# samyak0210/ViNet

Hardware: AMD Instinct MI355X
Metric: clips/sec training (32x224x384 bf16) (higher is better)
Workload: dtype bf16; 1 GPU; ViNet DHF1K training, 32x224x384 bf16, 192 clip(s)/GPU/step, kldiv + fused Adam, 1xMI355X; global_batch=192, local_batch=192, parallelism=dp1

## Files before the change

vinet_amd/csrc/options.h:

```cpp
#pragma once
#define VN_OPTIONS(VN_OPT) \
  VN_OPT(dma,          1, "LDS-DMA conv kernel (conv_dma) where legal; 0 = the register-staged kernel") \
  VN_OPT(dma3,         1, "LDS-DMA kernel for the split-bf16 form (conv_dma3); 0 = the register-staged kernel") \
  VN_OPT(pp,           1, "256x256x64 ping-pong conv kernel: 0 off, 1 heuristic, 2 force, 3 / 4 force the 256- / 192-wide shape") \
  VN_OPT(pp_pw_kt,     8, "ping-pong kernel on pointwise layers from this many K tiles of 64 (16 = as for every other layer)") \
  VN_OPT(pw,           1, "pointwise streaming kernel (conv_pw) for 1x1x1 convs and their data gradients: 0 off, 1 heuristic, 2 also on small grids (tests)") \
  VN_OPT(pw_maxtn,     4, "pointwise kernel: at most this many column tiles (each re-reads x)") \
  VN_OPT(ht,           1, "halo-tile conv kernels (conv_ht): 0 off, 1 heuristic, 2 every eligible conv (tests)") \
  VN_OPT(ht3,          1, "halo-tile kernels for the split-bf16 form; 0 = conv_dma3 everywhere") \
  VN_OPT(ht_minhw,     28 * 48, "halo tiles, spatial mode: smallest H x W the heuristic takes") \
  VN_OPT(ht_t,         1, "temporal mode of the halo-tile kernel for (3,1,1) / stride-1 convs; 0 off") \
  VN_OPT(ht_t_minhw,   14 * 24, "halo tiles, temporal mode: smallest H x W the heuristic takes") \
  VN_OPT(ht_pre,       0, "halo tiles, spatial mode, on inputs with a pending BatchNorm + ReLU: 1 on") \
  VN_OPT(conv_hs,      1, "strip-streaming kernel of the folded stem (conv_hs): 0 off, 1 heuristic, 2 every eligible shape (tests)") \
  VN_OPT(conv_hs_segs, 1, "conv_hs: row segments for launches on small grids; 0 = whole strips only") \
  VN_OPT(conv_ts,      1, "frame-streaming temporal 64 -> 64 kernels (conv_ts, conv_tsd): 0 off, 1 heuristic, 2 every eligible shape (tests)") \
  VN_OPT(conv_ts_segs, 1, "conv_ts: frame segments for launches on small grids; 0 = whole patches only") \
  VN_OPT(splitk,       1, "split-K on grids that cannot fill the chip: 0 off, 1 on, n >= 2 = minimum K chunks (of 32) per split") \
  VN_OPT(sk_tile,      7, "tiles of long-K small-grid convs whose caller lends split-K scratch: bit 0 128x192, bit 1 128x128, bit 2 / 3 128x64 / 256x64") \
  VN_OPT(n64_tile,     0, "tuning: 64-wide layers on 128x64 (1) or 64x64 (2) tiles instead of 256x64") \
  VN_OPT(n64_kmax,     64, "64-wide outputs: 128-row tiles up to this many K steps of 32 (0 = never)") \
  VN_OPT(n128_tile,    0, "tuning: 128-wide layers on 128x128 (1) or 64x128 (2) tiles instead of 256x128") \
  VN_OPT(n128_kmax,    64, "128-wide outputs: 128-row tiles up to this many K steps of 32 (0 = never)") \
  VN_OPT(n192_tile,    1, "128x192 tiles for N % 192 == 0 instead of 256x96: 0 off, 1 heuristic, 2 also on small grids (tests)") \
  VN_OPT(tperm,        0, "t-fastest M-tile order (L2 reuse across temporal taps): 1 on") \
  VN_OPT(epi_rows,     0, "conv epilogue stores whole rows through a wave-private LDS image: 1 on (-DVINET_EXPERIMENTS builds only)") \
  VN_OPT(bnb_epi,      1, "BatchNorm-backward partial sums out of the shared conv epilogue; 0 = only the fused temporal data gradient") \
  VN_OPT(wgrad_dma,    1, "LDS-DMA multi-tap weight-gradient kernel where legal; 0 = the register-staged kernel") \
  VN_OPT(wgrad_tg,     0, "tuning: taps per group in the LDS-DMA weight gradient (0 = heuristic)") \
  VN_OPT(wgrad_tr,     1, "hardware transpose reads in the register-staged weight gradient; 0 = scalar LDS reads") \
  VN_OPT(wgrad_pp,     1, "256x256x64 ping-pong weight gradient: 0 off, 1 heuristic, 2 force, 3 / 4 force the 256- / 192-row tile") \
  VN_OPT(wgrad_pp_cap, 1, "the ping-pong weight gradient honours VinetWgradDesc::max_cus; 0 = always the whole chip") \
  VN_OPT(wgrad_ts,     1, "frame-streaming weight gradient of temporal 64 -> 64 convs: 0 off, 1 heuristic, 2 every eligible shape (tests)") \
  VN_OPT(wgrad_ts_cap, 0, "the frame-streaming weight gradient honours VinetWgradDesc::max_cus: 1 on") \
  VN_OPT(wgrad_hs,     1, "strip-streaming weight gradient of the folded stem: 0 off, 1 heuristic, 2 every eligible shape (tests)") \
  VN_OPT(wgrad_rs,     1, "row-streaming weight gradient of 1x3x3 convs: 0 off, 1 heuristic, 2 every eligible shape (tests)") \
  VN_OPT(wgrad_rs4,    1, "row-streaming weight gradient: the four-wave form for W = 24, 48, 32, 64, 96; 0 = the eight-wave kernels") \
  VN_OPT(wgrad_tf,     1, "temporal-tap weight gradient (wgrad_tf): 0 off, 1 heuristic, 2 every eligible shape (tests)") \
  VN_OPT(wgrad_skinny, 1, "weight gradient of pointwise convs with 8 output channels: 0 off, 1 heuristic, 2 every eligible shape (tests)") \
  VN_OPT(bn_lean,      1, "register-lean bf16 BatchNorm-backward kernels: 0 = the generic 8-channel forms, 2 = a -DVINET_EXPERIMENTS variant") \
  VN_OPT(bn_rows,      1024, "cap on the workgroups (= partial rows) of a channel reduction (clamped to >= 1)") \
  VN_OPT(reduce_il,    1, "channel reductions: blocks interleave rounds over one window; 0 = one contiguous range per block") \
  VN_OPT(reduce_small, 1, "tensors of <= 64 voxels take channel_reduce_small_kernel; 0 off") \
  VN_OPT(pack_tiled,   1, "LDS-tiled multi-tensor pack / unpack; 0 = the element-wise kernels") \
  VN_OPT(pool_lds,     1, "LDS halo-tile 3x3x3/s1 max-pool forward (C % 64 == 0): 0 off, 1 large tensors, 2 always") \
  VN_OPT(pool_pk,      1, "bf16: packed 32-bit-key form of the LDS halo-tile pool; 0 = the fp32-compare kernel") \
  VN_OPT(pool_twalk,   1, "T-walking 3x3x3/s1 max-pool backward: 0 off, 1 large tensors, 2 always (any value above 3 too), 3 conditional-load form.  The forward's 8-channel T-walking kernel (kT 3, sT 1) reads it too: >= 2 forces it on small tensors, 0 does NOT switch it off") \
  VN_OPT(pool_blk,     1, "strided max-pool backward per 2x2 input block; 0 off") \
  VN_OPT(up_blk,       1, "8-channel upsample kernels (forward per 2x2 output block); 0 off") \
  VN_OPT(auc_ws,       0, "AUC-Judd sorts and counts in the caller's workspace whatever the number of fixations: 1 on (tests); 0 = in LDS up to 4096 fixations") \
  VN_OPT(sauc_ws,      0, "shuffled AUC reads the other-fixation list from the caller's workspace whatever its length: 1 on (tests); 0 = staged in LDS up to 8192 locations")

#define VN_OPT_DECLARE(name, dflt, text) extern int g_vinet_opt_##name;
VN_OPTIONS(VN_OPT_DECLARE)
```

vinet_amd/csrc/pool.hip:

```cpp
#include "elementwise.h"

struct PoolP { int kT, kH, kW, sT, sH, sW, pT, pH, pW; FastDiv dsT, dsH, dsW; };
static inline PoolP make_poolp(const VinetPoolDesc* d) {
  PoolP p = {d->kT, d->kH, d->kW, d->sT, d->sH, d->sW, d->pT, d->pH, d->pW, make_fastdiv((uint32_t)d->sT), make_fastdiv((uint32_t)d->sH), make_fastdiv((uint32_t)d->sW)};
  return p;
}

template <typename T> VN_DEV float pool_round(float v) { return v; }
template <> VN_DEV float pool_round<bf16_t>(float v) { return bf2f(f2bf(v)); }
template <typename T> VN_DEV float4 pool_pre4(float4 v, const Affine& pre, int c) {
  v = affine4(v, pre, c);
  if (pre.scale) { v.x = pool_round<T>(v.x); v.y = pool_round<T>(v.y); v.z = pool_round<T>(v.z); v.w = pool_round<T>(v.w); }
  return v;
}
template <typename T> VN_DEV float pool_pre(float f, float sc, float sh, const Affine& pre) {
  float v = fmaf(f, sc, sh);
  if (pre.relu) v = fmaxf(v, 0.f);
  if (pre.scale) v = pool_round<T>(v);
  return v;
}
VN_DEV void pool_column(const TView& v, uint32_t col, int& b, int& h, int& w) {
  const uint32_t r1 = fdiv(col, v.dW);
  w = (int)(col - r1 * (uint32_t)v.W);
  const uint32_t r2 = fdiv(r1, v.dH);
// ... 400 lines not shown
  const int h0 = th * 8, w0 = tw * 8, c0 = cg * 64 + oct * 8;
  const int ho = h0 + ph, wo = w0 + pw;
  const bool out_ok = ho < y.H && wo < y.W && c0 < x.C;
  const bool aff = pre.scale != nullptr;
  if (tid < 64) {
    const bool ok = aff && cg * 64 + tid < x.C;
    S[0][tid] = ok ? pre.scale[cg * 64 + tid] : 1.f;
    S[1][tid] = ok ? pre.shift[cg * 64 + tid] : 0.f;
  }
  __syncthreads();
  uint32_t m_a[8], m_b[8], m_c[8];
#pragma unroll
  for (int e = 0; e < 8; ++e) { m_a[e] = 0; m_b[e] = 0; m_c[e] = 0; }
  const int T_ = x.T;
  for (int tp = 0; tp <= T_; ++tp) {
    uint16_t (*buf)[64] = P[tp & 1];
    if (tp < T_) {
      for (int it = tid; it < 800; it += 512) {
        const int hp = it >> 3;
        const int hh = h0 - 1 + hp / 10, ww = w0 - 1 + hp % 10;
        if (cg * 64 + oct * 8 >= x.C) continue;
        uint4 q = make_uint4(0, 0, 0, 0);
        if ((unsigned)hh < (unsigned)x.H && (unsigned)ww < (unsigned)x.W) {
          q = *(const uint4*)((const bf16_t*)x.p + vox_off(x, b, tp, hh, ww) + cg * 64 + oct * 8);
          if (aff) {
            const float2* sp = (const float2*)&S[0][oct * 8];
            const float2* hp2 = (const float2*)&S[1][oct * 8];
            uint32_t* w4 = (uint32_t*)&q;
#pragma unroll
            for (int e = 0; e < 4; ++e) {
              const float2 s2 = sp[e], h2 = hp2[e];
              if (pre.relu) w4[e] = pre_relu_pair(w4[e], (f32x2_v){s2.x, s2.y}, (f32x2_v){h2.x, h2.y});
              else w4[e] = pack2bf(fmaf(__uint_as_float(w4[e] << 16), s2.x, h2.x), fmaf(__uint_as_float(w4[e] & 0xffff0000u), s2.y, h2.y));
            }
          } else if (pre.relu) {
            uint32_t* w4 = (uint32_t*)&q;
#pragma unroll
            for (int e = 0; e < 4; ++e) asm("v_pk_max_i16 %0, %1, 0" : "=v"(w4[e]) : "v"(w4[e]));
          }
          q.x = pool_code2(q.x); q.y = pool_code2(q.y); q.z = pool_code2(q.z); q.w = pool_code2(q.w);
        }
        *(uint4*)&buf[hp][oct * 8] = q;
      }
    }
    __syncthreads();
#pragma unroll
    for (int e = 0; e < 8; ++e) { m_a[e] = m_b[e]; m_b[e] = m_c[e]; m_c[e] = 0; }
    if (tp < T_) {
#pragma unroll
      for (int kh = 0; kh < 3; ++kh)
#pragma unroll
        for (int kw = 0; kw < 3; ++kw) {
          const uint4 q = *(const uint4*)&buf[(ph + kh) * 10 + pw + kw][oct * 8];
          const uint32_t ck = 8u - (uint32_t)(kh * 3 + kw);
          const uint32_t w4[4] = {q.x, q.y, q.z, q.w};
#pragma unroll
          for (int e = 0; e < 4; ++e) {
            const uint32_t klo = (w4[e] << 16) | ck, khi = (w4[e] & 0xffff0000u) | ck;
            m_c[2 * e] = m_c[2 * e] > klo ? m_c[2 * e] : klo;
            m_c[2 * e + 1] = m_c[2 * e + 1] > khi ? m_c[2 * e + 1] : khi;
          }
        }
    }
    const int to = tp - 1;
    if (to < 0 || !out_ok) continue;
    uint32_t ov[4];
    unsigned long long oi = 0;
    const bool va = to >= 1, vc = to + 1 < T_;
#pragma unroll
    for (int e = 0; e < 8; ++e) {
      const uint32_t ka = va ? m_a[e] + 18u : 0u, kb = m_b[e] + 9u, kc = vc ? m_c[e] : 0u;
      uint32_t k = ka > kb ? ka : kb;
      k = k > kc ? k : kc;
      if (e & 1) ov[e >> 1] |= k & 0xffff0000u; else ov[e >> 1] = k >> 16;
      oi |= (unsigned long long)(26u - (k & 0xffu)) << (8 * e);
    }
    uint4 o;
    o.x = pool_decode2(ov[0]); o.y = pool_decode2(ov[1]); o.z = pool_decode2(ov[2]); o.w = pool_decode2(ov[3]);
    *(uint4*)((bf16_t*)y.p + vox_off(y, b, to, ho, wo) + c0) = o;
    if (argmax) {
      const long ovox = (((long)b * y.T + to) * y.H + ho) * y.W + wo;
      *(unsigned long long*)(argmax + ovox * y.C + c0) = oi;
    }
  }
}

#define POOL_ADD_IF_X(g, word, BYTE, code, v, exec0)                                                                                  \
  asm volatile("v_cmpx_eq_u32_sdwa vcc, %1, %2 src0_sel:BYTE_" #BYTE " src1_sel:DWORD\n\tv_add_f32_e32 %0, %0, %3\n\ts_mov_b64 exec, %4" \
               : "+v"(g) : "v"(word), "s"(code), "v"(v), "s"(exec0) : "vcc")
#define POOL_ADD_IF(g, word, BYTE, code, v) POOL_ADD_IF_X(g, word, BYTE, code, v, exec0)
#define POOL_ADD_IF8(g, lo, hi, e, code, v, ex)                                           \
  do {                                                                                      \
    const uint32_t w_ = (e) < 4 ? (lo) : (hi);                                              \
    switch ((e) & 3) {                                                                      \
      case 0: POOL_ADD_IF_X(g, w_, 0, code, v, ex); break;                                  \
      case 1: POOL_ADD_IF_X(g, w_, 1, code, v, ex); break;                                  \
      case 2: POOL_ADD_IF_X(g, w_, 2, code, v, ex); break;                                  \
      default: POOL_ADD_IF_X(g, w_, 3, code, v, ex); break;                                 \
    }                                                                                       \
  } while (0)

template <typename T>
__global__ void maxpool_bwd_kernel(PoolP p, TView dy, const uint8_t* __restrict__ argmax, TView dx, int accumulate,
                                   long total) {
  const long i = (long)blockIdx.x * blockDim.x + threadIdx.x;
  if (i >= total) return;
  const uint32_t vox_u = fdiv((uint32_t)i, dx.dQ);
  const int q = (int)((uint32_t)i - vox_u * (uint32_t)(dx.C / 4));
  const long vox = (long)vox_u;
  int b, t, h, w;
  decode_vox(dx, vox, b, t, h, w);
  float g[4] = {0, 0, 0, 0};
  const int to1 = min((int)fdiv((uint32_t)(t + p.pT), p.dsT), dy.T - 1), ho1 = min((int)fdiv((uint32_t)(h + p.pH), p.dsH), dy.H - 1),
            wo1 = min((int)fdiv((uint32_t)(w + p.pW), p.dsW), dy.W - 1);
  const int to0 = (int)fdiv((uint32_t)max(0, t + p.pT - p.kT + p.sT), p.dsT), ho0 = (int)fdiv((uint32_t)max(0, h + p.pH - p.kH + p.sH), p.dsH),
            wo0 = (int)fdiv((uint32_t)max(0, w + p.pW - p.kW + p.sW), p.dsW);
  for (int to = to0; to <= to1; ++to) {
    const int kt = t + p.pT - to * p.sT;
    if (kt < 0 || kt >= p.kT) continue;
    for (int ho = ho0; ho <= ho1; ++ho) {
      const int kh = h + p.pH - ho * p.sH;
      if (kh < 0 || kh >= p.kH) continue;
      for (int wo = wo0; wo <= wo1; ++wo) {
        const int kw = w + p.pW - wo * p.sW;
        if (kw < 0 || kw >= p.kW) continue;
        const uint32_t tap = (uint32_t)((kt * p.kH + kh) * p.kW + kw);
        const long ovox = (((long)b * dy.T + to) * dy.H + ho) * dy.W + wo;
        const uint32_t am = *(const uint32_t*)(argmax + ovox * dy.C + q * 4);
        const uint32_t xr = am ^ (tap * 0x01010101u);
        if (!((xr - 0x01010101u) & ~xr & 0x80808080u)) continue;
        const float4 d = ldq<T>((const T*)dy.p + vox_off(dy, b, to, ho, wo) + q * 4);
        if ((xr & 0xffu) == 0) g[0] += d.x;
        if ((xr & 0xff00u) == 0) g[1] += d.y;
        if ((xr & 0xff0000u) == 0) g[2] += d.z;
        if ((xr & 0xff000000u) == 0) g[3] += d.w;
      }
    }
  }
  T* dst = (T*)dx.p + vox_off(dx, b, t, h, w) + q * 4;
  if (accumulate) { const float4 o = ldq<T>(dst); g[0] += o.x; g[1] += o.y; g[2] += o.z; g[3] += o.w; }
  stq<T>(dst, make_float4(g[0], g[1], g[2], g[3]));
}

template <typename T>
__global__ __launch_bounds__(256) void maxpool_bwd_k3s1_kernel(TView dy, const uint8_t* __restrict__ argmax, TView dx,
                                                               int accumulate, long total) {
  const long i = (long)blockIdx.x * blockDim.x + threadIdx.x;
  if (i >= total) return;
  const int G = dx.C >> 3;
  const uint32_t vox_u = (uint32_t)(i / G);
  const int g = (int)(i - (long)vox_u * G);
  int b, t, h, w;
  decode_vox(dx, (long)vox_u, b, t, h, w);
  const int T_ = dx.T, H = dx.H, W = dx.W;
  const long am_c = (long)vox_u * dx.C + g * 8;
  const long dy_c = vox_off(dy, b, t, h, w) + g * 8;
  unsigned long long am[27];
#pragma unroll
  for (int kt = 0; kt < 3; ++kt)
#pragma unroll
    for (int kh = 0; kh < 3; ++kh)
#pragma unroll
      for (int kw = 0; kw < 3; ++kw) {
        const int dt = 1 - kt, dh = 1 - kh, dw = 1 - kw;
        const bool ok = (unsigned)(t + dt) < (unsigned)T_ && (unsigned)(h + dh) < (unsigned)H && (unsigned)(w + dw) < (unsigned)W;
        const long d = ((long)(dt * H + dh) * W + dw) * (long)dx.C;
// ... 63 lines not shown
      }
    }
  }
  T* dst = (T*)dx.p + vox_off(dx, b, t, h, w) + g * 8;
  if (accumulate) {
    float o[8];
    ld8<T>(dst, o);
#pragma unroll
    for (int e = 0; e < 8; ++e) gr[e] += o[e];
  }
  st8<T>(dst, gr);
}

template <typename T>
__global__ __launch_bounds__(256) void maxpool_bwd_k133s2_kernel(TView dy, const uint8_t* __restrict__ argmax, TView dx, int accumulate,
                                                                 int HB, int WB, long total) {
  const long i = (long)blockIdx.x * blockDim.x + threadIdx.x;
  if (i >= total) return;
  const int G = dx.C >> 3;
  long r = i / G;
  const int g = (int)(i - r * G);
  const int wb = (int)(r % WB); r /= WB;
  const int hb = (int)(r % HB); r /= HB;
  const int t = (int)(r % dx.T);
  const int b = (int)(r / dx.T);
  const int h0 = 2 * hb, w0 = 2 * wb;
  unsigned long long am[4];
  bool wok[4];
#pragma unroll
  for (int q = 0; q < 4; ++q) {
    const int ho = hb + (q >> 1), wo = wb + (q & 1);
    wok[q] = ho < dy.H && wo < dy.W;
    const long ovox = (((long)b * dy.T + t) * dy.H + (wok[q] ? ho : 0)) * dy.W + (wok[q] ? wo : 0);
    am[q] = wok[q] ? *(const unsigned long long*)(argmax + ovox * dy.C + g * 8) : ~0ull;
  }
  float dv[4][8];
#pragma unroll
  for (int q = 0; q < 4; ++q) {
    bool any = false;
#pragma unroll
    for (int kh = 0; kh < 3; ++kh)
#pragma unroll
      for (int kw = 0; kw < 3; ++kw) {
        const bool in = ((q >> 1) ? kh == 0 : kh >= 1) && ((q & 1) ? kw == 0 : kw >= 1);
        if (!in) continue;
        const unsigned long long x = am[q] ^ ((unsigned long long)(kh * 3 + kw) * 0x0101010101010101ull);
        any |= ((x - 0x0101010101010101ull) & ~x & 0x8080808080808080ull) != 0;
      }
    if (any) ld8<T>((const T*)dy.p + vox_off(dy, b, t, hb + (q >> 1), wb + (q & 1)) + g * 8, dv[q]);
    else {
#pragma unroll
      for (int e = 0; e < 8; ++e) dv[q][e] = 0.f;
    }
  }
#pragma unroll
  for (int ih = 0; ih < 2; ++ih)
#pragma unroll
    for (int iw = 0; iw < 2; ++iw) {
      const int h = h0 + ih, w = w0 + iw;
      if (h >= dx.H || w >= dx.W) continue;
      float gr[8] = {0, 0, 0, 0, 0, 0, 0, 0};
      unsigned long long ex;
      asm volatile("s_mov_b64 %0, exec" : "=s"(ex));
#pragma unroll
      for (int q = 0; q < 4; ++q) {
        const int dh = q >> 1, dw = q & 1;
        const int kh = ih + 1 - 2 * dh, kw = iw + 1 - 2 * dw;
        if (kh < 0 || kw < 0) continue;
        const uint32_t alo = (uint32_t)am[q], ahi = (uint32_t)(am[q] >> 32);
#pragma unroll
        for (int e = 0; e < 8; ++e) POOL_ADD_IF8(gr[e], alo, ahi, e, (uint32_t)(kh * 3 + kw), dv[q][e], ex);
      }
      T* dst = (T*)dx.p + vox_off(dx, b, t, h, w) + g * 8;
      if (accumulate) {
        float o[8];
        ld8<T>(dst, o);
#pragma unroll
        for (int e = 0; e < 8; ++e) gr[e] += o[e];
      }
      st8<T>(dst, gr);
    }
}

template <typename T>
__global__ __launch_bounds__(256) void maxpool_bwd_k3s2_kernel(TView dy, const uint8_t* __restrict__ argmax, TView dx, int accumulate,
                                                               int TB, int HB, int WB, long total) {
  const long i = (long)blockIdx.x * blockDim.x + threadIdx.x;
  if (i >= total) return;
  const int G = dx.C >> 3;
  long r = i / G;
  const int g = (int)(i - r * G);
  const int wb = (int)(r % WB); r /= WB;
  const int hb = (int)(r % HB); r /= HB;
  const int tb = (int)(r % TB);
  const int b = (int)(r / TB);
  unsigned long long am[8];
  float dv[8][8];
#pragma unroll
  for (int w = 0; w < 8; ++w) {
    const int to = tb + (w >> 2), ho = hb + ((w >> 1) & 1), wo = wb + (w & 1);
    const bool ok = to < dy.T && ho < dy.H && wo < dy.W;
    am[w] = ~0ull;
    if (ok) {
      const long ovox = (((long)b * dy.T + to) * dy.H + ho) * dy.W + wo;
      am[w] = *(const unsigned long long*)(argmax + ovox * dy.C + g * 8);
      ld8<T>((const T*)dy.p + vox_off(dy, b, to, ho, wo) + g * 8, dv[w]);
    } else {
#pragma unroll
      for (int e = 0; e < 8; ++e) dv[w][e] = 0.f;
    }
  }
#pragma unroll
  for (int v = 0; v < 8; ++v) {
    const int it = v >> 2, ih = (v >> 1) & 1, iw = v & 1;
    const int t = 2 * tb + it, h = 2 * hb + ih, w_ = 2 * wb + iw;
    if (t >= dx.T || h >= dx.H || w_ >= dx.W) continue;
    float gr[8] = {0, 0, 0, 0, 0, 0, 0, 0};
    unsigned long long ex;
    asm volatile("s_mov_b64 %0, exec" : "=s"(ex));
#pragma unroll
    for (int w = 0; w < 8; ++w) {
      const int dt = w >> 2, dh = (w >> 1) & 1, dw = w & 1;
      if (dt > it || dh > ih || dw > iw) continue;
      const int kt = dt ? 0 : it + 1, kh = dh ? 0 : ih + 1, kw = dw ? 0 : iw + 1;
      const uint32_t alo = (uint32_t)am[w], ahi = (uint32_t)(am[w] >> 32);
#pragma unroll
      for (int e = 0; e < 8; ++e) POOL_ADD_IF8(gr[e], alo, ahi, e, (uint32_t)((kt * 3 + kh) * 3 + kw), dv[w][e], ex);
    }
    T* dst = (T*)dx.p + vox_off(dx, b, t, h, w_) + g * 8;
    if (accumulate) {
      float o[8];
      ld8<T>(dst, o);
#pragma unroll
      for (int e = 0; e < 8; ++e) gr[e] += o[e];
    }
    st8<T>(dst, gr);
  }
}

template <typename T>
__global__ __launch_bounds__(256) void maxpool_bwd_k3s1_twalk_kernel(TView dy, const uint8_t* __restrict__ argmax, TView dx,
                                                                     int accumulate, long total) {
  const long i = (long)blockIdx.x * blockDim.x + threadIdx.x;
  if (i >= total) return;
  const int G = dx.C >> 3;
  const uint32_t col = (uint32_t)(i / G);
  const int g = (int)(i - (long)col * G);
  int b, h, w;
  pool_column(dx, col, b, h, w);
  const int T_ = dx.T, H = dx.H, W = dx.W;
  float g_m[8], g_0[8], g_p[8];
#pragma unroll
  for (int e = 0; e < 8; ++e) { g_m[e] = 0.f; g_0[e] = 0.f; g_p[e] = 0.f; }
  for (int to = 0; to <= T_; ++to) {
    if (to < T_) {
      unsigned long long am[9];
#pragma unroll
      for (int kh = 0; kh < 3; ++kh)
#pragma unroll
        for (int kw = 0; kw < 3; ++kw) {
          const int ho = h + 1 - kh, wo = w + 1 - kw;
          const bool ok = (unsigned)ho < (unsigned)H && (unsigned)wo < (unsigned)W;
          const long ovox = (((long)b * T_ + to) * H + (ok ? ho : 0)) * W + (ok ? wo : 0);
          am[kh * 3 + kw] = ok ? *(const unsigned long long*)(argmax + ovox * dx.C + g * 8) : ~0ull;
        }
#pragma unroll
// ... 25 lines not shown
#pragma unroll
        for (int e = 0; e < 8; ++e) g_m[e] += o[e];
      }
      st8<T>(dst, g_m);
    }
#pragma unroll
    for (int e = 0; e < 8; ++e) { g_m[e] = g_0[e]; g_0[e] = g_p[e]; g_p[e] = 0.f; }
  }
}

__global__ __launch_bounds__(256) void maxpool_bwd_k3s1_tw3_kernel(TView dy, const uint8_t* __restrict__ argmax, TView dx,
                                                                   int accumulate, long total) {
  const long i = (long)blockIdx.x * blockDim.x + threadIdx.x;
  if (i >= total) return;
  unsigned long long exec0;
  asm volatile("s_mov_b64 %0, exec" : "=s"(exec0));
  const int G = dx.C >> 3;
  const uint32_t col = (uint32_t)(i / G);
  const int g = (int)(i - (long)col * G);
  int b, h, w;
  pool_column(dx, col, b, h, w);
  const int T_ = dx.T, H = dx.H, W = dx.W;
  const uint8_t* amp = argmax + ((((long)b * T_) * H + h) * W + w) * (long)dx.C + g * 8;
  const unsigned short* dyp = (const unsigned short*)dy.p + vox_off(dy, b, 0, h, w) + g * 8;
  const long am_plane = (long)H * W * dx.C, dy_plane = (long)H * W * dy.ld;
  uint32_t okmask = 0;
#pragma unroll
  for (int kh = 0; kh < 3; ++kh)
#pragma unroll
    for (int kw = 0; kw < 3; ++kw) {
      const int ho = h + 1 - kh, wo = w + 1 - kw;
      okmask |= (((unsigned)ho < (unsigned)H && (unsigned)wo < (unsigned)W) ? 1u : 0u) << (kh * 3 + kw);
    }
  float g_m[8], g_0[8], g_p[8];
#pragma unroll
  for (int e = 0; e < 8; ++e) { g_m[e] = 0.f; g_0[e] = 0.f; g_p[e] = 0.f; }
  for (int to = 0; to <= T_; ++to) {
    if (to < T_) {
      unsigned long long am[9];
      uint4 dv[9];
#pragma unroll
      for (int s = 0; s < 9; ++s) {
        const int dvox = (1 - s / 3) * W + (1 - s % 3);
        const bool ok = (okmask >> s) & 1u;
        am[s] = *(const unsigned long long*)(amp + (ok ? dvox * dx.C : 0));
        dv[s] = *(const uint4*)(dyp + (ok ? dvox * dy.ld : 0));
      }
#pragma unroll
      for (int s = 0; s < 9; ++s) {
        const unsigned long long a = ((okmask >> s) & 1u) ? am[s] : ~0ull;
        const uint32_t alo = (uint32_t)a, ahi = (uint32_t)(a >> 32);
        const uint32_t q[4] = {dv[s].x, dv[s].y, dv[s].z, dv[s].w};
#pragma unroll
        for (int e = 0; e < 8; ++e) {
          const uint32_t word = (e < 4) ? alo : ahi;
          const float v = (e & 1) ? __uint_as_float(q[e >> 1] & 0xffff0000u) : __uint_as_float(q[e >> 1] << 16);
          switch (e & 3) {
            case 0: POOL_ADD_IF(g_m[e], word, 0, (uint32_t)s, v); POOL_ADD_IF(g_0[e], word, 0, (uint32_t)(s + 9), v); POOL_ADD_IF(g_p[e], word, 0, (uint32_t)(s + 18), v); break;
            case 1: POOL_ADD_IF(g_m[e], word, 1, (uint32_t)s, v); POOL_ADD_IF(g_0[e], word, 1, (uint32_t)(s + 9), v); POOL_ADD_IF(g_p[e], word, 1, (uint32_t)(s + 18), v); break;
            case 2: POOL_ADD_IF(g_m[e], word, 2, (uint32_t)s, v); POOL_ADD_IF(g_0[e], word, 2, (uint32_t)(s + 9), v); POOL_ADD_IF(g_p[e], word, 2, (uint32_t)(s + 18), v); break;
            default: POOL_ADD_IF(g_m[e], word, 3, (uint32_t)s, v); POOL_ADD_IF(g_0[e], word, 3, (uint32_t)(s + 9), v); POOL_ADD_IF(g_p[e], word, 3, (uint32_t)(s + 18), v); break;
          }
        }
      }
      amp += am_plane;
      dyp += dy_plane;
    }
    const int t = to - 1;
    if (t >= 0) {
      unsigned short* dst = (unsigned short*)dx.p + vox_off(dx, b, t, h, w) + g * 8;
      if (accumulate) {
        float o[8];
        ld8<unsigned short>(dst, o);
#pragma unroll
        for (int e = 0; e < 8; ++e) g_m[e] += o[e];
      }
      st8<unsigned short>(dst, g_m);
    }
#pragma unroll
    for (int e = 0; e < 8; ++e) { g_m[e] = g_0[e]; g_0[e] = g_p[e]; g_p[e] = 0.f; }
  }
}

enum PoolKind { POOL_FWD, POOL_TSLIDE, POOL_FWD8, POOL_FWD8_PK, POOL_TSLIDE8, POOL_K3S1_LDS, POOL_K3S1_PK,
                POOL_BWD, POOL_BWD8, POOL_BWD_K133S2, POOL_BWD_K3S2, POOL_BWD_K3S1, POOL_BWD_K3S1_TWALK, POOL_BWD_K3S1_TW3 };
struct PoolRoute {
  PoolKind kind;
  const char* name;
  bool typed;
  long n;
  int tilesH, tilesW;
  int TB, HB, WB;
};

static const long POOL_FILL_COLS = 65536;

static bool pool_is_k3s1(const VinetPoolDesc* d, const VinetTensor& a, const VinetTensor& b) {
  return d->kT == 3 && d->kH == 3 && d->kW == 3 && d->sT == 1 && d->sH == 1 && d->sW == 1 && d->pT == 1 && d->pH == 1 && d->pW == 1 &&
         a.T == b.T && a.H == b.H && a.W == b.W;
}
static bool pool_oct(const VinetTensor& a, const VinetTensor& b, const uint8_t* argmax) {
  return oct_ok(a) && oct_ok(b) && ((uintptr_t)argmax % 8) == 0;
}

static PoolRoute pool_fwd_route(const VinetPoolDesc* d, const VinetTensor* x, VinetAffine pre, const VinetTensor* y, const uint8_t* argmax) {
  const bool oct = pool_oct(*x, *y, argmax);
  const bool walk_t = d->kT == 3 && d->sT == 1 && d->pT == 1 && y->T == x->T && x->T >= 2;
  const bool pk = d->dtype == VINET_BF16 && g_vinet_opt_pool_pk && (!pre.scale || pre.shift);
  const long cols8 = (long)y->B * y->H * y->W * (y->C / 8);
  if (pool_is_k3s1(d, *x, *y) && walk_t && oct && g_vinet_opt_pool_lds && (g_vinet_opt_pool_lds >= 2 || cols8 >= POOL_FILL_COLS)) {
    const int tilesH = (y->H + 7) / 8, tilesW = (y->W + 7) / 8;
    const long blocks = (long)y->B * tilesH * tilesW * ((y->C + 63) / 64);
    if (pk) return {POOL_K3S1_PK, "maxpool_k3s1_pk_kernel", false, blocks, tilesH, tilesW};
    return {POOL_K3S1_LDS, "maxpool_k3s1_lds_kernel", true, blocks, tilesH, tilesW};
  }
  if (walk_t && oct && (g_vinet_opt_pool_twalk >= 2 || cols8 >= POOL_FILL_COLS)) return {POOL_TSLIDE8, "maxpool_tslide8_kernel", true, cols8};
  if (walk_t && !(oct_ok(*x) && oct_ok(*y))) return {POOL_TSLIDE, "maxpool_tslide_kernel", true, (long)y->B * y->H * y->W * (y->C / 4)};
  if (oct) {
    const long total8 = view_voxels(*y) * (y->C / 8);
    if (pk) return {POOL_FWD8_PK, "maxpool_fwd8_pk_kernel", false, total8};
    return {POOL_FWD8, "maxpool_fwd8_kernel", true, total8};
  }
  return {POOL_FWD, "maxpool_fwd_kernel", true, view_voxels(*y) * (y->C / 4)};
}

static PoolRoute pool_bwd_route(const VinetPoolDesc* d, const VinetTensor* dy, const uint8_t* argmax, const VinetTensor* dx) {
  const bool oct = pool_oct(*dx, *dy, argmax);
  const long total8 = view_voxels(*dx) * (dx->C / 8);
  if (oct && pool_is_k3s1(d, *dx, *dy)) {
    const long cols8 = (long)dx->B * dx->H * dx->W * (dx->C / 8);
    if (g_vinet_opt_pool_twalk >= 2 || (g_vinet_opt_pool_twalk && cols8 >= POOL_FILL_COLS)) {
      if (g_vinet_opt_pool_twalk != 3 && d->dtype == VINET_BF16 && (long)dx->H * dx->W * dx->C < (1l << 30) &&
          (long)dx->H * dx->W * dy->ld < (1l << 30))
        return {POOL_BWD_K3S1_TW3, "maxpool_bwd_k3s1_tw3_kernel", false, cols8};
      return {POOL_BWD_K3S1_TWALK, "maxpool_bwd_k3s1_twalk_kernel", true, cols8};
    }
    return {POOL_BWD_K3S1, "maxpool_bwd_k3s1_kernel", true, total8};
  }
  if (oct && g_vinet_opt_pool_blk && d->kH == 3 && d->kW == 3 && d->sH == 2 && d->sW == 2 && d->pH == 1 && d->pW == 1 &&
      dy->H == (dx->H - 1) / 2 + 1 && dy->W == (dx->W - 1) / 2 + 1) {
    const int TB = (dx->T + 1) / 2, HB = (dx->H + 1) / 2, WB = (dx->W + 1) / 2;
    if (d->kT == 1 && d->sT == 1 && d->pT == 0 && dy->T == dx->T)
      return {POOL_BWD_K133S2, "maxpool_bwd_k133s2_kernel", true, (long)dx->B * dx->T * HB * WB * (dx->C / 8), 0, 0, 0, HB, WB};
    if (d->kT == 3 && d->sT == 2 && d->pT == 1 && dy->T == (dx->T - 1) / 2 + 1)
      return {POOL_BWD_K3S2, "maxpool_bwd_k3s2_kernel", true, (long)dx->B * TB * HB * WB * (dx->C / 8), 0, 0, TB, HB, WB};
  }
  if (oct) return {POOL_BWD8, "maxpool_bwd8_kernel", true, total8};
  return {POOL_BWD, "maxpool_bwd_kernel", true, view_voxels(*dx) * (dx->C / 4)};
}

static int pool_fwd_args(const VinetPoolDesc* d, const VinetTensor* x, const VinetTensor* y) {
  VN_CHECK_ARG(d && x && y && quad_ok(*x, esize(d->dtype)) && quad_ok(*y, esize(d->dtype)) && x->C == y->C && x->B == y->B,
               "maxpool3d: bad views");
  VN_CHECK_ARG(d->kT * d->kH * d->kW <= 255 && d->kT > 0 && d->kH > 0 && d->kW > 0, "maxpool3d: window too large");
  return 0;
}
static int pool_bwd_args(const VinetPoolDesc* d, const VinetTensor* dy, const uint8_t* argmax, const VinetTensor* dx) {
  VN_CHECK_ARG(d && dy && dx && argmax && quad_ok(*dy, esize(d->dtype)) && quad_ok(*dx, esize(d->dtype)) &&
                   dx->C == dy->C && dx->B == dy->B, "maxpool3d_bwd: bad views");
  return 0;
}
static int pool_kernel_name(const PoolRoute& r, int dtype, char* buf, int32_t n) {
  snprintf(buf, n, r.typed ? "%s<%s>" : "%s", r.name, dtype == VINET_F32 ? "f32" : "bf16");
  return 0;
}

extern "C" int vinet_maxpool3d_kernel_name(const VinetPoolDesc* d, const VinetTensor* x, VinetAffine pre, const VinetTensor* y,
                                           const uint8_t* argmax, char* buf, int32_t n) {
  if (!buf || n <= 0 || pool_fwd_args(d, x, y)) return -1;
  return pool_kernel_name(pool_fwd_route(d, x, pre, y, argmax), d->dtype, buf, n);
}
extern "C" int vinet_maxpool3d_bwd_kernel_name(const VinetPoolDesc* d, const VinetTensor* dy, const uint8_t* argmax,
                                               const VinetTensor* dx, char* buf, int32_t n) {
  if (!buf || n <= 0 || pool_bwd_args(d, dy, argmax, dx)) return -1;
  return pool_kernel_name(pool_bwd_route(d, dy, argmax, dx), d->dtype, buf, n);
}

extern "C" int vinet_maxpool3d(const VinetPoolDesc* d, const VinetTensor* x, VinetAffine pre, const VinetTensor* y,
                               uint8_t* argmax, void* stream) {
  if (pool_fwd_args(d, x, y)) return -1;
  const PoolRoute r = pool_fwd_route(d, x, pre, y, argmax);
  const PoolP p = make_poolp(d);
  const TView xv = make_view(*x), yv = make_view(*y);
  const Affine a = make_affine(pre);
  const hipStream_t s = (hipStream_t)stream;
  const dim3 lanes(256), grid(r.kind == POOL_K3S1_PK || r.kind == POOL_K3S1_LDS ? (unsigned)r.n : ew_grid(r.n));
  switch (r.kind) {
    case POOL_K3S1_PK: hipLaunchKernelGGL(maxpool_k3s1_pk_kernel, grid, dim3(512), 0, s, xv, a, yv, argmax, r.tilesH, r.tilesW); break;
    case POOL_K3S1_LDS:
      DISPATCH_T(d->dtype, T, hipLaunchKernelGGL(maxpool_k3s1_lds_kernel<T>, grid, dim3(512), 0, s, xv, a, yv, argmax,
                                                 r.tilesH, r.tilesW);) break;
    case POOL_TSLIDE8:
      DISPATCH_T(d->dtype, T, hipLaunchKernelGGL(maxpool_tslide8_kernel<T>, grid, lanes, 0, s, p, xv, a, yv, argmax, r.n);) break;
    case POOL_TSLIDE:
      DISPATCH_T(d->dtype, T, hipLaunchKernelGGL(maxpool_tslide_kernel<T>, grid, lanes, 0, s, p, xv, a, yv, argmax, r.n);) break;
    case POOL_FWD8_PK: hipLaunchKernelGGL(maxpool_fwd8_pk_kernel, grid, lanes, 0, s, p, xv, a, yv, argmax, r.n); break;
    case POOL_FWD8:
      DISPATCH_T(d->dtype, T, hipLaunchKernelGGL(maxpool_fwd8_kernel<T>, grid, lanes, 0, s, p, xv, a, yv, argmax, r.n);) break;
    case POOL_FWD:
      DISPATCH_T(d->dtype, T, hipLaunchKernelGGL(maxpool_fwd_kernel<T>, grid, lanes, 0, s, p, xv, a, yv, argmax, r.n);) break;
    default: break;
  }
  return vn_launch_status(r.name);
}

extern "C" int vinet_maxpool3d_bwd(const VinetPoolDesc* d, const VinetTensor* dy, const uint8_t* argmax,
                                   const VinetTensor* dx, int32_t accumulate, void* stream) {
  if (pool_bwd_args(d, dy, argmax, dx)) return -1;
  const PoolRoute r = pool_bwd_route(d, dy, argmax, dx);
  const PoolP p = make_poolp(d);
  const TView gv = make_view(*dy), xv = make_view(*dx);
  const hipStream_t s = (hipStream_t)stream;
  const dim3 lanes(256), grid(ew_grid(r.n));
  switch (r.kind) {
    case POOL_BWD_K3S1_TW3: hipLaunchKernelGGL(maxpool_bwd_k3s1_tw3_kernel, grid, lanes, 0, s, gv, argmax, xv, accumulate, r.n); break;
    case POOL_BWD_K3S1_TWALK:
      DISPATCH_T(d->dtype, T, hipLaunchKernelGGL(maxpool_bwd_k3s1_twalk_kernel<T>, grid, lanes, 0, s, gv, argmax, xv, accumulate, r.n);) break;
    case POOL_BWD_K3S1:
      DISPATCH_T(d->dtype, T, hipLaunchKernelGGL(maxpool_bwd_k3s1_kernel<T>, grid, lanes, 0, s, gv, argmax, xv, accumulate, r.n);) break;
    case POOL_BWD_K133S2:
      DISPATCH_T(d->dtype, T, hipLaunchKernelGGL(maxpool_bwd_k133s2_kernel<T>, grid, lanes, 0, s, gv, argmax, xv, accumulate,
                                                 r.HB, r.WB, r.n);) break;
    case POOL_BWD_K3S2:
      DISPATCH_T(d->dtype, T, hipLaunchKernelGGL(maxpool_bwd_k3s2_kernel<T>, grid, lanes, 0, s, gv, argmax, xv, accumulate,
                                                 r.TB, r.HB, r.WB, r.n);) break;
    case POOL_BWD8:
      DISPATCH_T(d->dtype, T, hipLaunchKernelGGL(maxpool_bwd8_kernel<T>, grid, lanes, 0, s, p, gv, argmax, xv, accumulate, r.n);) break;
    case POOL_BWD:
      DISPATCH_T(d->dtype, T, hipLaunchKernelGGL(maxpool_bwd_kernel<T>, grid, lanes, 0, s, p, gv, argmax, xv, accumulate, r.n);) break;
    default: break;
  }
  return vn_launch_status(r.name);
}
```

Baseline: 703.4 clips/s.

## Add LDS halo-tile kernels for bf16 1x3x3 stride-2 max-pool forward and backward

Adds tiled max-pool kernels for the bf16 1x3x3 / stride (1,2,2) pool, used on large tensors. The forward stages a (2TR+1)x(2TW+1) input halo per 64-channel group in LDS, applying the pending affine/ReLU and key encoding once per input voxel instead of per window tap. The backward stages the dy and argmax window in LDS so each 2x2 input block reads its neighbours' gradients from shared memory. The aim is to cut redundant global reads of overlapping windows, at the cost of a block barrier, LDS use, and one more routing path.

New measurement: 710.0 clips/s (median of 6 runs). About the same (+0.9%).

```diff
diff --git a/vinet_amd/csrc/options.h b/vinet_amd/csrc/options.h
--- a/vinet_amd/csrc/options.h
+++ b/vinet_amd/csrc/options.h
@@ -43,7 +43,7 @@
   VN_OPT(reduce_il,    1, "channel reductions: blocks interleave rounds over one window; 0 = one contiguous range per block") \
   VN_OPT(reduce_small, 1, "tensors of <= 64 voxels take channel_reduce_small_kernel; 0 off") \
   VN_OPT(pack_tiled,   1, "LDS-tiled multi-tensor pack / unpack; 0 = the element-wise kernels") \
-  VN_OPT(pool_lds,     1, "LDS halo-tile 3x3x3/s1 max-pool forward (C % 64 == 0): 0 off, 1 large tensors, 2 always") \
+  VN_OPT(pool_lds,     1, "LDS halo-tile max-pool kernels, the 3x3x3/s1 forward and the bf16 1x3x3/s(1,2,2) forward and backward: 0 off, 1 large tensors, 2 always") \
   VN_OPT(pool_pk,      1, "bf16: packed 32-bit-key form of the LDS halo-tile pool; 0 = the fp32-compare kernel") \
   VN_OPT(pool_twalk,   1, "T-walking 3x3x3/s1 max-pool backward: 0 off, 1 large tensors, 2 always (any value above 3 too), 3 conditional-load form.  The forward's 8-channel T-walking kernel (kT 3, sT 1) reads it too: >= 2 forces it on small tensors, 0 does NOT switch it off") \
   VN_OPT(pool_blk,     1, "strided max-pool backward per 2x2 input block; 0 off") \
diff --git a/vinet_amd/csrc/pool.hip b/vinet_amd/csrc/pool.hip
--- a/vinet_amd/csrc/pool.hip
+++ b/vinet_amd/csrc/pool.hip
@@ -506,6 +506,107 @@
       const long ovox = (((long)b * y.T + to) * y.H + ho) * y.W + wo;
       *(unsigned long long*)(argmax + ovox * y.C + c0) = oi;
     }
+  }
+}
+
+#ifndef POOL_TILE_TR
+#define POOL_TILE_TR 4
+#endif
+#ifndef POOL_TILE_TW
+#define POOL_TILE_TW 16
+#endif
+#define POOL_STR_(x) #x
+#define POOL_STR(x) POOL_STR_(x)
+#define POOL_TILE_NAME(k) k "<" POOL_STR(POOL_TILE_TR) "," POOL_STR(POOL_TILE_TW) ">"
+
+template <int TR, int TW>
+__global__ __launch_bounds__(TR * TW * 8) void maxpool_k133s2_tile_kernel(TView x, Affine pre, TView y, uint8_t* __restrict__ argmax,
+                                                                          int tilesH, int tilesW) {
+  constexpr int NT = TR * TW * 8, PH = 2 * TR + 1, PW = 2 * TW + 1, NPOS = PH * PW, NIT = (NPOS * 8 + NT - 1) / NT;
+  __shared__ __attribute__((aligned(16))) uint16_t P[NPOS][64];
+  const int tid = threadIdx.x;
+  const int oct = tid & 7, pos = tid >> 3;
+  const int ph = pos / TW, pw = pos % TW;
+  int bid = blockIdx.x;
+  const int ncg = (x.C + 63) >> 6;
+  const int cg = bid % ncg; bid /= ncg;
+  const int tw = bid % tilesW; bid /= tilesW;
+  const int th = bid % tilesH; bid /= tilesH;
+  const int t = bid % x.T;
+  const int b = bid / x.T;
+  const int c0 = cg * 64 + oct * 8;
+  const bool c_ok = c0 < x.C;
+  const bool aff = pre.scale != nullptr;
+  f32x2_v sc2[4], sh2[4];
+#pragma unroll
+  for (int e = 0; e < 4; ++e) {
+    sc2[e] = aff && c_ok ? (f32x2_v){pre.scale[c0 + 2 * e], pre.scale[c0 + 2 * e + 1]} : (f32x2_v){1.f, 1.f};
+    sh2[e] = aff && c_ok ? (f32x2_v){pre.shift[c0 + 2 * e], pre.shift[c0 + 2 * e + 1]} : (f32x2_v){0.f, 0.f};
+  }
+  const int hb = 2 * th * TR - 1, wb = 2 * tw * TW - 1;
+  uint4 q[NIT];
+  bool in[NIT];
+#pragma unroll
+  for (int k = 0; k < NIT; ++k) {
+    const int hp = (tid + k * NT) >> 3;
+    const int hh = hb + hp / PW, ww = wb + hp % PW;
+    in[k] = hp < NPOS && c_ok && (unsigned)hh < (unsigned)x.H && (unsigned)ww < (unsigned)x.W;
+    q[k] = make_uint4(0, 0, 0, 0);
+    if (in[k]) q[k] = *(const uint4*)((const bf16_t*)x.p + vox_off(x, b, t, hh, ww) + c0);
+  }
+#pragma unroll
+  for (int k = 0; k < NIT; ++k) {
+    const int hp = (tid + k * NT) >> 3;
+    if (in[k]) {
+      uint32_t* w4 = (uint32_t*)&q[k];
+#pragma unroll
+      for (int e = 0; e < 4; ++e) {
+        if (aff) {
+          if (pre.relu) w4[e] = pre_relu_pair(w4[e], sc2[e], sh2[e]);
+          else w4[e] = pack2bf(fmaf(__uint_as_float(w4[e] << 16), sc2[e].x, sh2[e].x), fmaf(__uint_as_float(w4[e] & 0xffff0000u), sc2[e].y, sh2[e].y));
+        } else if (pre.relu) {
+          asm("v_pk_max_i16 %0, %1, 0" : "=v"(w4[e]) : "v"(w4[e]));
+        }
+        w4[e] = pool_code2(w4[e]);
+      }
+    }
+    if (hp < NPOS) *(uint4*)&P[hp][oct * 8] = q[k];
+  }
+  __syncthreads();
+  const int ho = th * TR + ph, wo = tw * TW + pw;
+  if (!c_ok || ho >= y.H || wo >= y.W) return;
+  uint32_t best[8];
+#pragma unroll
+  for (int e = 0; e < 8; ++e) best[e] = 0;
+#pragma unroll
+  for (int kh = 0; kh < 3; ++kh)
+#pragma unroll
+    for (int kw = 0; kw < 3; ++kw) {
+      const bool ok = (unsigned)(2 * ho - 1 + kh) < (unsigned)x.H && (unsigned)(2 * wo - 1 + kw) < (unsigned)x.W;
+      const uint32_t ck = ok ? 8u - (uint32_t)(kh * 3 + kw) : 0u;
+      const uint4 v = *(const uint4*)&P[(2 * ph + kh) * PW + 2 * pw + kw][oct * 8];
+      const uint32_t w4[4] = {v.x, v.y, v.z, v.w};
+#pragma unroll
+      for (int e = 0; e < 4; ++e) {
+        const uint32_t klo = (w4[e] << 16) | ck, khi = (w4[e] & 0xffff0000u) | ck;
+        best[2 * e] = best[2 * e] > klo ? best[2 * e] : klo;
+        best[2 * e + 1] = best[2 * e + 1] > khi ? best[2 * e + 1] : khi;
+      }
+    }
+  uint32_t ov[4];
+  unsigned long long bi = 0;
+#pragma unroll
+  for (int e = 0; e < 8; ++e) {
+    const uint32_t k = best[e];
+    if (e & 1) ov[e >> 1] |= k & 0xffff0000u; else ov[e >> 1] = k >> 16;
+    bi |= (unsigned long long)(8u - (k & 0xffu)) << (8 * e);
+  }
+  uint4 o;
+  o.x = pool_decode2(ov[0]); o.y = pool_decode2(ov[1]); o.z = pool_decode2(ov[2]); o.w = pool_decode2(ov[3]);
+  *(uint4*)((bf16_t*)y.p + vox_off(y, b, t, ho, wo) + c0) = o;
+  if (argmax) {
+    const long ovox = (((long)b * y.T + t) * y.H + ho) * y.W + wo;
+    *(unsigned long long*)(argmax + ovox * y.C + c0) = bi;
   }
 }
 
@@ -735,6 +836,92 @@
     }
 }
 
+template <int TR, int TW>
+__global__ __launch_bounds__(TR * TW * 8) void maxpool_bwd_k133s2_tile_kernel(TView dy, const uint8_t* __restrict__ argmax, TView dx,
+                                                                              int accumulate, int tilesH, int tilesW) {
+  constexpr int NT = TR * TW * 8, WH = TR + 1, WW = TW + 1, NWIN = WH * WW, NIT = (NWIN * 8 + NT - 1) / NT;
+  __shared__ __attribute__((aligned(16))) uint4 D[NWIN][8];
+  __shared__ __attribute__((aligned(8))) unsigned long long A[NWIN][8];
+  const int tid = threadIdx.x;
+  const int oct = tid & 7, pos = tid >> 3;
+  const int ph = pos / TW, pw = pos % TW;
+  int bid = blockIdx.x;
+  const int ncg = (dx.C + 63) >> 6;
+  const int cg = bid % ncg; bid /= ncg;
+  const int tw = bid % tilesW; bid /= tilesW;
+  const int th = bid % tilesH; bid /= tilesH;
+  const int t = bid % dx.T;
+  const int b = bid / dx.T;
+  const int c0 = cg * 64 + oct * 8;
+  const bool c_ok = c0 < dx.C;
+  const int hb = th * TR + ph, wb = tw * TW + pw;
+  const int h0 = 2 * hb, w0 = 2 * wb;
+  const bool lane_ok = c_ok && h0 < dx.H && w0 < dx.W;
+  uint4 old[4];
+#pragma unroll
+  for (int v = 0; v < 4; ++v) {
+    old[v] = make_uint4(0, 0, 0, 0);
+    if (accumulate && lane_ok && h0 + (v >> 1) < dx.H && w0 + (v & 1) < dx.W)
+      old[v] = ld16_nt((const bf16_t*)dx.p + vox_off(dx, b, t, h0 + (v >> 1), w0 + (v & 1)) + c0);
+  }
+  unsigned long long sa[NIT];
+  uint4 sd[NIT];
+#pragma unroll
+  for (int k = 0; k < NIT; ++k) {
+    const int wp = (tid + k * NT) >> 3;
+    const int ho = th * TR + wp / WW, wo = tw * TW + wp % WW;
+    sa[k] = ~0ull;
+    sd[k] = make_uint4(0, 0, 0, 0);
+    if (wp < NWIN && c_ok && ho < dy.H && wo < dy.W) {
+      const long ovox = (((long)b * dy.T + t) * dy.H + ho) * dy.W + wo;
+      sa[k] = *(const unsigned long long*)(argmax + ovox * dy.C + c0);
+      sd[k] = *(const uint4*)((const bf16_t*)dy.p + vox_off(dy, b, t, ho, wo) + c0);
+    }
+  }
+#pragma unroll
+  for (int k = 0; k < NIT; ++k) {
+    const int wp = (tid + k * NT) >> 3;
+    if (wp < NWIN) { A[wp][oct] = sa[k]; D[wp][oct] = sd[k]; }
+  }
+  __syncthreads();
+  if (!lane_ok) return;
+  unsigned long long am[4];
+  float dv[4][8];
+#pragma unroll
+  for (int q = 0; q < 4; ++q) {
+    const int wp = (ph + (q >> 1)) * WW + pw + (q & 1);
+    am[q] = A[wp][oct];
+    unpack16<bf16_t>(D[wp][oct], dv[q]);
+  }
+#pragma unroll
+  for (int ih = 0; ih < 2; ++ih)
+#pragma unroll
+    for (int iw = 0; iw < 2; ++iw) {
+      const int h = h0 + ih, w = w0 + iw;
+      if (h >= dx.H || w >= dx.W) continue;
+      float gr[8] = {0, 0, 0, 0, 0, 0, 0, 0};
+      unsigned long long ex;
+      asm volatile("s_mov_b64 %0, exec" : "=s"(ex));
+#pragma unroll
+      for (int q = 0; q < 4; ++q) {
+        const int dh = q >> 1, dw = q & 1;
+        const int kh = ih + 1 - 2 * dh, kw = iw + 1 - 2 * dw;
+        if (kh < 0 || kw < 0) continue;
+        const uint32_t alo = (uint32_t)am[q], ahi = (uint32_t)(am[q] >> 32);
+#pragma unroll
+        for (int e = 0; e < 8; ++e) POOL_ADD_IF8(gr[e], alo, ahi, e, (uint32_t)(kh * 3 + kw), dv[q][e], ex);
+      }
+      bf16_t* dst = (bf16_t*)dx.p + vox_off(dx, b, t, h, w) + c0;
+      if (accumulate) {
+        float o[8];
+        unpack16<bf16_t>(old[ih * 2 + iw], o);
+#pragma unroll
+        for (int e = 0; e < 8; ++e) gr[e] += o[e];
+      }
+      st8_nt<bf16_t>(dst, gr);
+    }
+}
+
 template <typename T>
 __global__ __launch_bounds__(256) void maxpool_bwd_k3s2_kernel(TView dy, const uint8_t* __restrict__ argmax, TView dx, int accumulate,
                                                                int TB, int HB, int WB, long total) {
@@ -926,8 +1113,8 @@
   }
 }
 
-enum PoolKind { POOL_FWD, POOL_TSLIDE, POOL_FWD8, POOL_FWD8_PK, POOL_TSLIDE8, POOL_K3S1_LDS, POOL_K3S1_PK,
-                POOL_BWD, POOL_BWD8, POOL_BWD_K133S2, POOL_BWD_K3S2, POOL_BWD_K3S1, POOL_BWD_K3S1_TWALK, POOL_BWD_K3S1_TW3 };
+enum PoolKind { POOL_FWD, POOL_TSLIDE, POOL_FWD8, POOL_FWD8_PK, POOL_TSLIDE8, POOL_K3S1_LDS, POOL_K3S1_PK, POOL_K133S2_TILE,
+                POOL_BWD, POOL_BWD8, POOL_BWD_K133S2, POOL_BWD_K133S2_TILE, POOL_BWD_K3S2, POOL_BWD_K3S1, POOL_BWD_K3S1_TWALK, POOL_BWD_K3S1_TW3 };
 struct PoolRoute {
   PoolKind kind;
   const char* name;
@@ -945,6 +1132,20 @@
 }
 static bool pool_oct(const VinetTensor& a, const VinetTensor& b, const uint8_t* argmax) {
   return oct_ok(a) && oct_ok(b) && ((uintptr_t)argmax % 8) == 0;
+}
+
+static const long POOL_TILE_LANES = 1l << 23;
+static bool pool_is_k133s2(const VinetPoolDesc* d, const VinetTensor& in, const VinetTensor& out) {
+  return d->kT == 1 && d->kH == 3 && d->kW == 3 && d->sT == 1 && d->sH == 2 && d->sW == 2 && d->pT == 0 && d->pH == 1 && d->pW == 1 &&
+         out.T == in.T && out.H == (in.H - 1) / 2 + 1 && out.W == (in.W - 1) / 2 + 1;
+}
+static bool pool_tile_grid(const VinetPoolDesc* d, const VinetTensor& in, int H, int W, PoolRoute& r) {
+  const long lanes = (long)in.B * in.T * H * W * (in.C / 8);
+  if (d->dtype != VINET_BF16 || !g_vinet_opt_pool_lds || (g_vinet_opt_pool_lds < 2 && lanes < POOL_TILE_LANES)) return false;
+  r.tilesH = (H + POOL_TILE_TR - 1) / POOL_TILE_TR;
+  r.tilesW = (W + POOL_TILE_TW - 1) / POOL_TILE_TW;
+  r.n = (long)in.B * in.T * r.tilesH * r.tilesW * ((in.C + 63) / 64);
+  return r.n < (1l << 31);
 }
 
 static PoolRoute pool_fwd_route(const VinetPoolDesc* d, const VinetTensor* x, VinetAffine pre, const VinetTensor* y, const uint8_t* argmax) {
@@ -960,6 +1161,10 @@
   }
   if (walk_t && oct && (g_vinet_opt_pool_twalk >= 2 || cols8 >= POOL_FILL_COLS)) return {POOL_TSLIDE8, "maxpool_tslide8_kernel", true, cols8};
   if (walk_t && !(oct_ok(*x) && oct_ok(*y))) return {POOL_TSLIDE, "maxpool_tslide_kernel", true, (long)y->B * y->H * y->W * (y->C / 4)};
+  if (oct && pk && pool_is_k133s2(d, *x, *y)) {
+    PoolRoute r = {POOL_K133S2_TILE, POOL_TILE_NAME("maxpool_k133s2_tile_kernel"), false, 0};
+    if (pool_tile_grid(d, *x, y->H, y->W, r)) return r;
+  }
   if (oct) {
     const long total8 = view_voxels(*y) * (y->C / 8);
     if (pk) return {POOL_FWD8_PK, "maxpool_fwd8_pk_kernel", false, total8};
@@ -984,8 +1189,11 @@
   if (oct && g_vinet_opt_pool_blk && d->kH == 3 && d->kW == 3 && d->sH == 2 && d->sW == 2 && d->pH == 1 && d->pW == 1 &&
       dy->H == (dx->H - 1) / 2 + 1 && dy->W == (dx->W - 1) / 2 + 1) {
     const int TB = (dx->T + 1) / 2, HB = (dx->H + 1) / 2, WB = (dx->W + 1) / 2;
-    if (d->kT == 1 && d->sT == 1 && d->pT == 0 && dy->T == dx->T)
+    if (d->kT == 1 && d->sT == 1 && d->pT == 0 && dy->T == dx->T) {
+      PoolRoute r = {POOL_BWD_K133S2_TILE, POOL_TILE_NAME("maxpool_bwd_k133s2_tile_kernel"), false, 0};
+      if (pool_tile_grid(d, *dx, HB, WB, r)) return r;
       return {POOL_BWD_K133S2, "maxpool_bwd_k133s2_kernel", true, (long)dx->B * dx->T * HB * WB * (dx->C / 8), 0, 0, 0, HB, WB};
+    }
     if (d->kT == 3 && d->sT == 2 && d->pT == 1 && dy->T == (dx->T - 1) / 2 + 1)
       return {POOL_BWD_K3S2, "maxpool_bwd_k3s2_kernel", true, (long)dx->B * TB * HB * WB * (dx->C / 8), 0, 0, TB, HB, WB};
   }
@@ -1028,8 +1236,12 @@
   const TView xv = make_view(*x), yv = make_view(*y);
   const Affine a = make_affine(pre);
   const hipStream_t s = (hipStream_t)stream;
-  const dim3 lanes(256), grid(r.kind == POOL_K3S1_PK || r.kind == POOL_K3S1_LDS ? (unsigned)r.n : ew_grid(r.n));
+  const dim3 lanes(256), grid(r.kind == POOL_K3S1_PK || r.kind == POOL_K3S1_LDS || r.kind == POOL_K133S2_TILE ? (unsigned)r.n : ew_grid(r.n));
   switch (r.kind) {
+    case POOL_K133S2_TILE:
+      hipLaunchKernelGGL((maxpool_k133s2_tile_kernel<POOL_TILE_TR, POOL_TILE_TW>), grid, dim3(POOL_TILE_TR * POOL_TILE_TW * 8), 0, s, xv, a, yv,
+                         argmax, r.tilesH, r.tilesW);
+      break;
     case POOL_K3S1_PK: hipLaunchKernelGGL(maxpool_k3s1_pk_kernel, grid, dim3(512), 0, s, xv, a, yv, argmax, r.tilesH, r.tilesW); break;
     case POOL_K3S1_LDS:
       DISPATCH_T(d->dtype, T, hipLaunchKernelGGL(maxpool_k3s1_lds_kernel<T>, grid, dim3(512), 0, s, xv, a, yv, argmax,
@@ -1055,8 +1267,12 @@
   const PoolP p = make_poolp(d);
   const TView gv = make_view(*dy), xv = make_view(*dx);
   const hipStream_t s = (hipStream_t)stream;
-  const dim3 lanes(256), grid(ew_grid(r.n));
+  const dim3 lanes(256), grid(r.kind == POOL_BWD_K133S2_TILE ? (unsigned)r.n : ew_grid(r.n));
   switch (r.kind) {
+    case POOL_BWD_K133S2_TILE:
+      hipLaunchKernelGGL((maxpool_bwd_k133s2_tile_kernel<POOL_TILE_TR, POOL_TILE_TW>), grid, dim3(POOL_TILE_TR * POOL_TILE_TW * 8), 0, s, gv,
+                         argmax, xv, accumulate, r.tilesH, r.tilesW);
+      break;
     case POOL_BWD_K3S1_TW3: hipLaunchKernelGGL(maxpool_bwd_k3s1_tw3_kernel, grid, lanes, 0, s, gv, argmax, xv, accumulate, r.n); break;
     case POOL_BWD_K3S1_TWALK:
       DISPATCH_T(d->dtype, T, hipLaunchKernelGGL(maxpool_bwd_k3s1_twalk_kernel<T>, grid, lanes, 0, s, gv, argmax, xv, accumulate, r.n);) break;
```
